# federicobetti99/Conjugate-Gradient

Measured on AMD Instinct MI355X. Metric: cg_iterations_per_sec, higher is better.
Workload: dtype f64

## Files before the change

conjugate-gradient_amd/cgx.py:

```python
import ctypes as C
import os
import subprocess
import sys

import numpy as np

_PKG = os.path.dirname(os.path.abspath(__file__))
LIB_PATH = os.path.join(_PKG, "libcgx.so")
UNIQUE_ID_BYTES = 128

IPC_HANDLE_BYTES = 64
COMM_SELF, COMM_LOOPBACK, COMM_RCCL, COMM_P2P = 0, 1, 2, 3
MATRIX_DENSE, MATRIX_BANDED = 0, 1
MATRIX_CSR = 2
MAX_DIAGONALS = 64

EXPORTS = [
    "cgx_config_init", "cgx_comm_unique_id", "cgx_create", "cgx_destroy", "cgx_last_error", "cgx_status_string",
    "cgx_get_comm_info", "cgx_get_gemv_plan", "cgx_get_resident_record", "cgx_p2p_export", "cgx_p2p_import", "cgx_p2p_selftest",
    "cgx_partition", "cgx_generate_lap2d_matrix", "cgx_set_matrix_dense", "cgx_read_matrix",
    "cgx_init_source_term", "cgx_set_source_term", "cgx_set_max_iter", "cgx_set_tolerance", "cgx_get_size",
    "cgx_get_matrix_format",
    "cgx_solve", "cgx_solve_begin", "cgx_solve_steps", "cgx_solve_end", "cgx_get_gemv_samples",
    "cgx_get_update_samples",
    "cgx_probe_gemv", "cgx_probe_time_gemv", "cgx_probe_vector_ops", "cgx_probe_get_matrix_rows",
    "cgx_probe_get_source_term", "cgx_probe_set_fault_after", "cgx_probe_set_resident_limit", "cgx_probe_persistent_plan",
    "cgx_probe_parse_matrix_market", "cgx_probe_p2p_mailbox_to_host", "cgx_probe_fill_matrix_hash",
    "cgx_probe_set_p2p_epoch", "cgx_probe_get_p2p_epoch", "cgx_probe_p2p_host_mailboxes", "cgx_probe_resident_test",
    "cgx_solve_multi", "cgx_probe_gemv_multi",
    "cgx_set_preconditioner", "cgx_get_preconditioner",
    "cgx_set_preconditioner_block", "cgx_get_preconditioner_block", "cgx_probe_get_precond_blocks",
    "cgx_set_matrix_csr", "cgx_get_matrix_nnz",
]
MAX_RHS = 16
PRECOND_NONE, PRECOND_JACOBI = 0, 1
_PRECOND_NAMES = {None: PRECOND_NONE, "jacobi": PRECOND_JACOBI}
PRECOND_BLOCKS = (1, 2, 4, 8, 16, 32, 64, 128, 256)


class Config(C.Structure):
    _fields_ = [
        ("struct_version", C.c_int), ("comm_mode", C.c_int), ("device", C.c_int), ("rank", C.c_int),
        ("nranks", C.c_int), ("unique_id", C.c_ubyte * UNIQUE_ID_BYTES), ("gemv_variant", C.c_int),
        ("lda_pad", C.c_int), ("check_every", C.c_int), ("profile_gemv", C.c_int), ("profile_update", C.c_int),
        ("p2p_mailbox_kib", C.c_int), ("p2p_timeout_ms", C.c_int), ("p2p_separate_exchange", C.c_int),
        ("matrix_format", C.c_int), ("profile_first", C.c_int), ("profile_markers", C.c_int),
        ("p2p_no_acquire_fence", C.c_int), ("p2p_tagged", C.c_int),
    ]


class Result(C.Structure):
    _fields_ = [
# ... 20 lines not shown
    subprocess.check_call(args)
    return LIB_PATH


_lib = None


def lib():
    global _lib
    if _lib is None:
        if not os.path.exists(LIB_PATH):
            raise OSError("libcgx.so not built (run `make -C conjugate-gradient_amd` or __graft_entry__.build()); "
                          "the product path has no CPU fallback")
        if "torch" not in sys.modules and os.environ.get("CGX_NO_TORCH") != "1":
            try:
                import torch
            except Exception:
                pass
        L = C.CDLL(LIB_PATH)
        dp = C.POINTER(C.c_double)
        ip = C.POINTER(C.c_int)
        vp = C.c_void_p
        L.cgx_config_init.argtypes = [C.POINTER(Config)]
        L.cgx_config_init.restype = None
        L.cgx_comm_unique_id.argtypes = [C.POINTER(C.c_ubyte)]
        L.cgx_create.argtypes = [C.POINTER(vp), C.POINTER(Config)]
        L.cgx_destroy.argtypes = [vp]
        L.cgx_last_error.argtypes = [vp]
        L.cgx_last_error.restype = C.c_char_p
        L.cgx_status_string.argtypes = [C.c_int]
        L.cgx_status_string.restype = C.c_char_p
        L.cgx_get_comm_info.argtypes = [vp, ip, ip, ip, C.c_char_p]
        L.cgx_get_gemv_plan.argtypes = [vp, C.c_int, ip]
        L.cgx_get_resident_record.argtypes = [vp, C.POINTER(C.c_longlong)]
        L.cgx_p2p_export.argtypes = [vp, C.POINTER(C.c_ubyte)]
        L.cgx_p2p_import.argtypes = [vp, C.POINTER(C.c_ubyte)]
        L.cgx_p2p_selftest.argtypes = [vp, C.c_int, ip]
        L.cgx_partition.argtypes = [C.c_int, C.c_int, ip, ip]
        L.cgx_generate_lap2d_matrix.argtypes = [vp, C.c_int]
        L.cgx_set_matrix_dense.argtypes = [vp, dp, C.c_long, C.c_int]
        L.cgx_read_matrix.argtypes = [vp, C.c_char_p]
        L.cgx_init_source_term.argtypes = [vp, C.c_double]
        L.cgx_set_source_term.argtypes = [vp, dp]
        L.cgx_set_max_iter.argtypes = [vp, C.c_int]
        L.cgx_set_tolerance.argtypes = [vp, C.c_double]
        L.cgx_get_size.argtypes = [vp, ip, ip]
        L.cgx_get_matrix_format.argtypes = [vp, C.c_int, ip, ip, ip, dp]
        L.cgx_set_matrix_csr.argtypes = [vp, C.c_int, C.POINTER(C.c_longlong), ip, dp]
        L.cgx_get_matrix_nnz.argtypes = [vp, C.c_int, C.POINTER(C.c_longlong)]
        L.cgx_solve.argtypes = [vp, dp, C.POINTER(Result)]
        L.cgx_solve_begin.argtypes = [vp, dp]
        L.cgx_solve_steps.argtypes = [vp, C.c_int, ip]
        L.cgx_solve_end.argtypes = [vp, dp, C.POINTER(Result)]
        L.cgx_get_gemv_samples.argtypes = [vp, dp, C.c_int, ip]
        L.cgx_get_update_samples.argtypes = [vp, dp, C.c_int, ip]
        L.cgx_probe_gemv.argtypes = [vp, dp, dp, dp]
        L.cgx_probe_time_gemv.argtypes = [vp, C.c_int, dp]
        L.cgx_probe_vector_ops.argtypes = [vp, C.c_int, C.c_double, C.c_double, dp, dp, dp, dp, dp]
        L.cgx_probe_get_matrix_rows.argtypes = [vp, C.c_int, dp, ip, ip]
        L.cgx_probe_get_source_term.argtypes = [vp, C.c_int, dp]
        L.cgx_probe_set_fault_after.argtypes = [vp, C.c_int]
        L.cgx_probe_set_resident_limit.argtypes = [vp, C.c_int]
        L.cgx_probe_persistent_plan.argtypes = [C.c_int, C.c_int, C.c_long, C.c_int, C.POINTER(C.c_long)]
        L.cgx_probe_p2p_mailbox_to_host.argtypes = [vp]
        L.cgx_probe_fill_matrix_hash.argtypes = [vp, C.c_ulonglong, C.c_int, C.c_double]
        L.cgx_probe_p2p_host_mailboxes.argtypes = [vp, C.c_char_p, C.c_int]
# ... 95 lines not shown
    def _check(self, st):
        if st:
            raise CgxError(st, lib().cgx_last_error(self._h).decode(errors="replace"))

    def close(self):
        if getattr(self, "_h", None) and self._h.value:
            lib().cgx_destroy(self._h)
            self._h = C.c_void_p()

    def __del__(self):
        try:
            self.close()
        except Exception:
            pass

    def __enter__(self):
        return self

    def __exit__(self, *exc):
        self.close()

    def comm_info(self):
        mode, wired, seen = C.c_int(), C.c_int(), C.c_int()
        dev = C.create_string_buffer(32)
        self._check(lib().cgx_get_comm_info(self._h, C.byref(mode), C.byref(wired), C.byref(seen), dev))
        return {"comm_mode": mode.value, "ranks_wired": wired.value, "rank_seen": seen.value,
                "device_id": dev.value.decode(errors="replace")}

    def gemv_plan(self, local_shard=0):
        v = (C.c_int * 8)()
        self._check(lib().cgx_get_gemv_plan(self._h, int(local_shard), v))
        return dict(zip(("variant", "R", "U", "waves", "light", "split", "grid", "ncols"), list(v)))

    def resident_record(self):
        v = (C.c_longlong * 10)()
        self._check(lib().cgx_get_resident_record(self._h, v))
        return dict(zip(("iterations", "watch_repeats", "gather_repeats", "launches", "wg0_first_wait_ticks", "wg0_longest_wait_ticks",
                         "max_first_wait_ticks", "max_longest_wait_ticks", "fallbacks", "persistent"), list(v)))

    def p2p_export(self):
        buf = (C.c_ubyte * IPC_HANDLE_BYTES)()
        self._check(lib().cgx_p2p_export(self._h, buf))
        return bytes(buf)

    def p2p_import(self, handles):
        assert len(handles) == self.nranks * IPC_HANDLE_BYTES
        buf = (C.c_ubyte * len(handles)).from_buffer_copy(handles)
        self._check(lib().cgx_p2p_import(self._h, buf))

    def p2p_selftest(self, rounds=32):
        ok = C.c_int()
        self._check(lib().cgx_p2p_selftest(self._h, int(rounds), C.byref(ok)))
        return bool(ok.value)

    def matrix_format(self, local_shard=0):
        fmt, nd, nbytes = C.c_int(), C.c_int(), C.c_double()
        offs = (C.c_int * MAX_DIAGONALS)()
        self._check(lib().cgx_get_matrix_format(self._h, int(local_shard), C.byref(fmt), C.byref(nd), offs, C.byref(nbytes)))
        return fmt.value, list(offs[:nd.value]), nbytes.value

    def matrix_nnz(self, local_shard=0):
        nnz = C.c_longlong()
        self._check(lib().cgx_get_matrix_nnz(self._h, int(local_shard), C.byref(nnz)))
        return nnz.value

    def set_matrix_csr(self, indptr, indices=None, data=None, n=None):
# ... 189 lines not shown
```

conjugate-gradient_amd/csrc/cgx_context.cpp:

```cpp
#include "cgx_internal.h"

#include <sys/mman.h>
#include <sys/stat.h>
#include <fcntl.h>
#include <unistd.h>

#include <algorithm>
#include <cctype>
#include <chrono>
#include <cmath>
#include <cstdio>
#include <cstdlib>
#include <cstring>
#include <string>
#include <vector>

using namespace cgxi;

namespace cgxi {

constexpr int kStreamDefaultMax = 10000;

thread_local std::string g_create_error;

// ... 25 lines not shown
void bind_state(Shard &s, long lda)
{
    double *b = s.state[s.cur];
    s.x = b;
    s.rbuf = b + cgx::state_off_r(lda);
    s.p[1] = b + cgx::state_off_p(lda);
    s.sc = reinterpret_cast<Scalars *>(b + cgx::state_off_sc(lda));
    s.rv.base = s.rbuf;
}

void free_shard(Shard &s)
{
    if (s.state[0]) {
        (void)hipFree(s.state[0]);
        (void)hipFree(s.state[1]);
        s.x = s.p[1] = s.rbuf = nullptr;
        s.sc = nullptr;
    }
    (void)hipFree(s.A);
    (void)hipFree(s.dia_vals);
    (void)hipFree(s.csr_rp);
    (void)hipFree(s.csr_col);
    (void)hipFree(s.csr_vals);
    (void)hipFree(s.b_full);
    (void)hipFree(s.x);
    (void)hipFree(s.p[0]);
    (void)hipFree(s.p[1]);
    (void)hipFree(s.apg);
    (void)hipFree(s.rbuf);
    (void)hipFree(s.partials);
    (void)hipFree(s.ap_parts);
    (void)hipFree(s.k1_scratch);
    (void)hipFree(s.sym_parts);
    (void)hipFree(s.dinv);
    (void)hipFree(s.W);
    (void)hipFree(s.zbuf);
    (void)hipFree(s.sc);
    (void)hipFree(s.gathered);
    s = Shard{};
}

void free_problem(cgx_ctx *ctx)
{
    for (auto &s : ctx->shards) free_shard(s);
    ctx->shards.clear();
    (void)hipFree(ctx->d_gathered_ptrs);
    (void)hipFree(ctx->d_scalar_ptrs);
    (void)hipFree(ctx->multi);
    ctx->multi = nullptr;
    ctx->multi_bytes = 0;
    if (ctx->h_stage) (void)hipHostFree(ctx->h_stage);
    ctx->h_stage = nullptr;
    ctx->d_gathered_ptrs = nullptr;
    ctx->d_scalar_ptrs = nullptr;
    ctx->have_matrix = ctx->have_b = false;
    ctx->in_solve = false;
    ctx->dinv_valid = false;
    (void)hipFree(ctx->d_jbad);
    ctx->d_jbad = nullptr;
}

static long p2p_flag_bytes() { return (long)cgx::kP2pChannels * cgx::kMaxRanks * cgx::kP2pFlagStride; }
static long p2p_data0_off() { return p2p_flag_bytes() + (long)cgx::kMaxChunkFlags * 8; }
long p2p_fixed_prefix(int nranks)
{
    return p2p_data0_off() + 2L * nranks * 16 + 2L * nranks * (long)cgx::kSlots * 8;
// ... 246 lines not shown
        }
        if (ctx->chunked) {
            HIP_TRY(ctx, hipMalloc(&s.k1_scratch, (size_t)(grid_max + 8) * sizeof(double)));
            HIP_TRY(ctx, hipMemsetAsync(s.k1_scratch, 0, (size_t)(grid_max + 8) * sizeof(double), ctx->stream));
        }
        if (!blocks) HIP_TRY(ctx, hipMalloc(&s.sc, sizeof(Scalars)));
        HIP_TRY(ctx, hipMalloc(&s.gathered, (size_t)cgx::kMaxRanks * cgx::kSlots * sizeof(double)));
        HIP_TRY(ctx, hipMemsetAsync(s.p[0], 0, (size_t)ctx->lda * sizeof(double), ctx->stream));
        HIP_TRY(ctx, hipMemsetAsync(s.p[1], 0, (size_t)ctx->lda * sizeof(double), ctx->stream));
        HIP_TRY(ctx, hipMemsetAsync(s.apg, 0, apg_bytes, ctx->stream));
        HIP_TRY(ctx, hipMemsetAsync(s.rbuf, 0, rbuf_bytes, ctx->stream));
        if (s.rows <= 0 && s.A) HIP_TRY(ctx, hipMemsetAsync(s.A, 0, (size_t)ctx->lda * sizeof(double), ctx->stream));
        HIP_TRY(ctx, hipMemsetAsync(s.partials, 0, (size_t)s.npartials * sizeof(double), ctx->stream));
        HIP_TRY(ctx, hipMemsetAsync(s.sc, 0, sizeof(Scalars), ctx->stream));
        HIP_TRY(ctx, hipMemsetAsync(s.gathered, 0, (size_t)cgx::kMaxRanks * cgx::kSlots * sizeof(double), ctx->stream));
    }
    CGX_TRY(setup_resident(ctx, variant));
    if (ctx->cfg.comm_mode == CGX_COMM_LOOPBACK) {
        std::vector<double *> gp(nlocal);
        std::vector<Scalars *> sp(nlocal);
        for (int i = 0; i < nlocal; ++i) {
            gp[i] = ctx->shards[i].gathered;
            sp[i] = ctx->shards[i].sc;
        }
        HIP_TRY(ctx, hipMalloc(&ctx->d_gathered_ptrs, nlocal * sizeof(double *)));
        HIP_TRY(ctx, hipMalloc(&ctx->d_scalar_ptrs, nlocal * sizeof(Scalars *)));
        HIP_TRY(ctx, hipMemcpy(ctx->d_gathered_ptrs, gp.data(), nlocal * sizeof(double *), hipMemcpyHostToDevice));
        HIP_TRY(ctx, hipMemcpy(ctx->d_scalar_ptrs, sp.data(), nlocal * sizeof(Scalars *), hipMemcpyHostToDevice));
    }
    HIP_TRY(ctx, hipStreamSynchronize(ctx->stream));
    return CGX_OK;
}

cgx_status plan_symmetric(cgx_ctx *ctx)
{
    ctx->dinv_valid = false;
    if (ctx->shards.size() != 1 || ctx->nranks != 1 || ctx->sparse() || ctx->chunked) return CGX_OK;
    Shard &s = ctx->shards[0];
    int variant = ctx->cfg.gemv_variant;
    if (variant <= 0) {
        const char *e = getenv("CGX_GEMV_VARIANT");
        if (e) variant = atoi(e);
    }
    const int k1_variant = (variant == 40000 || variant == 50000) ? 0 : variant;
    const cgx::GemvPlan general = cgx::plan_gemv(k1_variant, s.rows, ctx->n, ctx->lda, false);
    const cgx::GemvPlan sym = cgx::plan_symv(ctx->n, ctx->lda, ctx->cus);
    const bool eligible = variant <= 0 && ctx->n > cgx::kSymvMinN && s.rows == ctx->n && s.A && sym.light <= ctx->npart;
    if (!eligible) {
        s.plan = general;
        return CGX_OK;
    }
    DeviceScratch scratch;
    int *dflag = nullptr;
    HIP_TRY(ctx, scratch.alloc(&dflag, sizeof(int)));
    HIP_TRY(ctx, hipMemsetAsync(dflag, 0, sizeof(int), ctx->stream));
    HIP_TRY(ctx, cgx::launch_symmetric_check(s.A, ctx->lda, ctx->n, dflag, ctx->stream));
    int mismatch = 1;
    HIP_TRY(ctx, hipMemcpyAsync(&mismatch, dflag, sizeof(int), hipMemcpyDeviceToHost, ctx->stream));
    HIP_TRY(ctx, hipStreamSynchronize(ctx->stream));
    if (mismatch) {
        s.plan = general;
        return CGX_OK;
    }
    const size_t bytes = (size_t)sym.split * (size_t)ctx->lda * sizeof(double);
    if (s.sym_parts && s.sym_parts_bytes != bytes) {
        (void)hipFree(s.sym_parts);
        s.sym_parts = nullptr;
        s.sym_parts_bytes = 0;
    }
    if (!s.sym_parts) {
        HIP_TRY(ctx, hipMalloc(&s.sym_parts, bytes));
        s.sym_parts_bytes = bytes;
        HIP_TRY(ctx, hipMemsetAsync(s.sym_parts, 0, bytes, ctx->stream));
        HIP_TRY(ctx, hipStreamSynchronize(ctx->stream));
    }
    s.plan = sym;
    return CGX_OK;
}

}

extern "C" {

void cgx_config_init(cgx_config *cfg)
{
    if (!cfg) return;
    memset(cfg, 0, sizeof *cfg);
    cfg->struct_version = CGX_VERSION;
    cfg->comm_mode = CGX_COMM_SELF;
    cfg->device = 0;
    cfg->rank = 0;
    cfg->nranks = 1;
    cfg->lda_pad = -1;
}

const char *cgx_status_string(cgx_status s)
{
    switch (s) {
    case CGX_OK: return "ok";
    case CGX_ERR_BAD_ARG: return "bad argument";
    case CGX_ERR_IO: return "i/o error";
    case CGX_ERR_HIP: return "HIP error";
    case CGX_ERR_RCCL: return "RCCL error";
    case CGX_ERR_OOM: return "out of memory";
    case CGX_ERR_NO_DEVICE: return "no usable GPU (libcgx has no CPU fallback)";
    case CGX_ERR_UNSUPPORTED: return "unsupported input";
    case CGX_ERR_P2P: return "direct peer exchange failed";
    }
    return "unknown";
}
// ... 149 lines not shown
        break;
    case CGX_COMM_LOOPBACK:
        wired = ctx->nranks;
        break;
    default:
        break;
    }
    if (comm_mode) *comm_mode = ctx->cfg.comm_mode;
    if (ranks_wired) *ranks_wired = wired;
    if (rank_seen) *rank_seen = seen;
    if (device_id) {
        device_id[0] = 0;
        HIP_TRY(ctx, hipDeviceGetPCIBusId(device_id, 32, ctx->device));
    }
    return CGX_OK;
}

cgx_status cgx_get_gemv_plan(const cgx_ctx *ctx, int local_shard, int out[CGX_GEMV_PLAN_INTS])
{
    if (!ctx || !out || local_shard < 0 || local_shard >= (int)ctx->shards.size()) return CGX_ERR_BAD_ARG;
    const cgx::GemvPlan &pl = ctx->shards[(size_t)local_shard].plan;
    if (ctx->resident && ctx->rplan.stream) {
        const int r[CGX_GEMV_PLAN_INTS] = {5, ctx->rplan.R, ctx->rplan.S, 8, ctx->rplan.RB, ctx->rplan.RL + ctx->rplan.RG, ctx->rplan.grid, pl.ncols};
        memcpy(out, r, sizeof r);
        return CGX_OK;
    }
    if (ctx->resident) {
        const int r[CGX_GEMV_PLAN_INTS] = {4, ctx->rplan.R, ctx->rplan.S, 4, ctx->rplan.RG, 1, ctx->rplan.grid, pl.ncols};
        memcpy(out, r, sizeof r);
        return CGX_OK;
    }
    const int v[CGX_GEMV_PLAN_INTS] = {pl.variant, pl.R, pl.U, pl.waves, pl.light, pl.split, pl.grid, pl.ncols};
    memcpy(out, v, sizeof v);
    return CGX_OK;
}

cgx_status cgx_get_resident_record(const cgx_ctx *ctx, long long out[CGX_RESIDENT_RECORD_INTS])
{
    if (!ctx || !out) return CGX_ERR_BAD_ARG;
    for (int i = 0; i < 8; ++i) out[i] = ctx->res_rec[i];
    out[8] = ctx->res_fallbacks;
    out[9] = ctx->resident ? 1 : 0;
    return CGX_OK;
}

cgx_status cgx_p2p_export(cgx_ctx *ctx, unsigned char out[CGX_IPC_HANDLE_BYTES])
{
    static_assert(sizeof(hipIpcMemHandle_t) == CGX_IPC_HANDLE_BYTES, "hipIpcMemHandle_t size");
    if (!ctx || !out || ctx->cfg.comm_mode != CGX_COMM_P2P) return fail(ctx, CGX_ERR_BAD_ARG, "cgx_p2p_export: not a P2P context");
    HIP_TRY(ctx, hipSetDevice(ctx->device));
    hipIpcMemHandle_t h;
    HIP_TRY(ctx, hipIpcGetMemHandle(&h, ctx->mailbox));
    memcpy(out, &h, CGX_IPC_HANDLE_BYTES);
    return CGX_OK;
}

cgx_status cgx_p2p_import(cgx_ctx *ctx, const unsigned char *handles)
{
    if (!ctx || !handles || ctx->cfg.comm_mode != CGX_COMM_P2P) return fail(ctx, CGX_ERR_BAD_ARG, "cgx_p2p_import: not a P2P context");
    HIP_TRY(ctx, hipSetDevice(ctx->device));
    for (int q = 0; q < ctx->nranks; ++q) {
        if (q == ctx->cfg.rank) continue;
        hipIpcMemHandle_t h;
        memcpy(&h, handles + (size_t)q * CGX_IPC_HANDLE_BYTES, CGX_IPC_HANDLE_BYTES);
        void *ptr = nullptr;
        hipError_t e = hipIpcOpenMemHandle(&ptr, h, hipIpcMemLazyEnablePeerAccess);
// ... 216 lines not shown
```

conjugate-gradient_amd/csrc/cgx_internal.h:

```cpp
#pragma once

#include "../../include/cgx.h"

#include <hip/hip_runtime.h>

#include <string>
#include <vector>

#include "cgx_kernels.h"
#include "cgx_rccl.h"

namespace cgxi {

using cgx::Scalars;

struct Shard {
    int rank = 0;
    int row0 = 0;
    int rows = 0;
    double *A = nullptr;
    double *dia_vals = nullptr;
    cgx::DiaView dia{};
    long long *csr_rp = nullptr;
    int *csr_col = nullptr;
    double *csr_vals = nullptr;
    cgx::CsrView csr{};
    double *b_full = nullptr;
    double *state[2] = {nullptr, nullptr};
    int cur = 0;
    double *x = nullptr;
    double *p[2] = {nullptr, nullptr};
    double *apg = nullptr;
    double *rbuf = nullptr;
    double *ap_parts = nullptr;
    double *k1_scratch = nullptr;
    double *partials = nullptr;
    double *sym_parts = nullptr;
    size_t sym_parts_bytes = 0;
    Scalars *sc = nullptr;
    double *gathered = nullptr;
    cgx::GemvPlan plan{};
    cgx::SegView apv{}, rv{};
    double *dinv = nullptr;
    double *zbuf = nullptr;
    double *W = nullptr;
    int w_block = 0;
    cgx::SegView zv{};
    int npartials = 0;
    double *Ap() const { return apg + (size_t)rank * apv.S; }
    double *tail() const { return Ap() + apv.Sr; }
    double *k1_part() const { return k1_scratch ? k1_scratch : tail(); }
};


}

struct cgx_ctx {
    cgx_config cfg{};
    int device = 0;
    hipStream_t stream = nullptr;
    int nranks = 1;
    int m = 0, n = 0;
    long lda = 0;
    int max_iter = 0;
    double tol = 1e-10;
    std::vector<int> start_rows, num_rows;
    std::vector<cgxi::Shard> shards;
    std::vector<double> b_host;
    bool have_matrix = false, have_b = false;
    bool banded = false;
    bool csr = false;
// ... 192 lines not shown
```

conjugate-gradient_amd/csrc/cgx_kernels.h:

```cpp
#pragma once

#include <hip/hip_runtime.h>

namespace cgx {

constexpr int kSlots = 4;
constexpr int kSlotConj = 0;
constexpr int kSlotRr = 1;
constexpr int kSlotX = 2;
constexpr int kMaxRanks = 64;

struct Scalars {
    double rs[2];
    double rr[2];
    double local[kSlots];
    double dbg[4];
    int    done;
    int    k_final;
    unsigned pad[2];
};

struct SegView {
    double *base;
    int S, Sr;
// ... 8 lines not shown
void seg_finalize(SegView *sv);

struct GemvPlan {
    int variant;
    int R;
    int U;
    int waves;
    int nt;
    int grid;
    int rows_per_wg;
    int ncols;
    int split;
    int light;
};

GemvPlan plan_gemv(int variant, int rows, int n, long lda, bool allow_split = false);

hipError_t launch_gemv_plain(const GemvPlan &plan, const double *A, long lda, int rows, const double *v_full,
                             const double *v_local, double *Ap, double *partials, Scalars *sc, hipStream_t s);

hipError_t launch_gemv_fused(const GemvPlan &plan, const double *A, long lda, int rows, int row0,
                             const double *p_old, double *p_new, SegView seg, double *Ap, double *partials,
                             Scalars *sc, int k, double tol, hipStream_t s, hipEvent_t e_start = nullptr,
                             hipEvent_t e_stop = nullptr, long ap_stride = 0, bool jacobi = false);
constexpr int kSymvTile = 256;
constexpr int kSymvMinN = 16384;
GemvPlan plan_symv(int n, long lda, int cus);
inline int plan_partials(const GemvPlan &pl) { return pl.variant == 6 ? pl.light : pl.grid / (pl.split > 1 ? pl.split : 1); }
hipError_t launch_symv_plain(const GemvPlan &pl, const double *A, long lda, int n, const double *v, double *parts, double *Ap,
                             double *partials, hipStream_t s);
hipError_t launch_symv_fused(const GemvPlan &pl, const double *A, long lda, int n, const double *p_old, double *p_new, SegView seg,
                             double *parts, double *Ap, double *partials, Scalars *sc, int k, double tol, hipStream_t s,
                             hipEvent_t e_start = nullptr, hipEvent_t e_stop = nullptr, bool jacobi = false);
hipError_t launch_symmetric_check(const double *A, long lda, int n, int *mismatch, hipStream_t s);

constexpr int kChunkRows = 512;
inline int chunks_per_rank(int Sr) { return (Sr + kChunkRows - 1) / kChunkRows; }
hipError_t launch_prefold_ap(const double *parts, int split, long stride, int rows, int Sr, const double *p_loc, double *dst,
                             double *tail, const Scalars *sc, hipStream_t s);

hipError_t launch_update_xr(int n, int rows, int row0, const double *p_new, SegView apv, int tail_off, int tail_count,
                            double *x, SegView rv, Scalars *sc, int parity, double *partials, hipStream_t s,
                            hipEvent_t e_start = nullptr, hipEvent_t e_stop = nullptr,
                            const double *dinv = nullptr, SegView zv = SegView{},
                            const double *W = nullptr, int block = 1, long lda = 0);
int update_xr_grid(int count);
constexpr int kMaxVectorGrid = 1024;

hipError_t launch_close_iteration(Scalars *sc, SegView seg, int k, double tol, hipStream_t s, bool jacobi = false);

hipError_t launch_reduce_partials(const double *partials, int n, double *out, hipStream_t s);
hipError_t launch_reduce_partials3(const double *partials, int n, double *out3, hipStream_t s);

hipError_t launch_init_residual(int n, const double *b_full, SegView apv, SegView rv, double *partials, hipStream_t s,
                                const double *dinv = nullptr, SegView zv = SegView{}, const double *W = nullptr, int block = 1,
                                long lda = 0);

hipError_t launch_diag_slice(const double *A, long lda, int rows, int row0, double *dst, hipStream_t s);
hipError_t launch_jacobi_dinv(SegView apv, int n, long lda, double *dinv, int *bad, hipStream_t s);

constexpr int kBjMaxBlock = 256;
constexpr int kBjLdsBlock = 128;
bool bj_block_ok(int block);
hipError_t launch_bj_col_slice(const double *A, long lda, int n, int rows, int row0, int block, int t0, int nt, double *dst,
                               long dst_stride, hipStream_t s);
hipError_t launch_bj_invert(double *W, long lda, int n, int block, int *bad, hipStream_t s);
// ... 196 lines not shown
```

conjugate-gradient_amd/csrc/cgx_solve.cpp:

```cpp
#include "cgx_internal.h"

#include <sys/file.h>

#include <cerrno>
#include <climits>
#include <thread>

#include <algorithm>
#include <cctype>
#include <chrono>
#include <cmath>
#include <cstdio>
#include <cstdlib>
#include <cstring>
#include <string>
#include <vector>

using namespace cgxi;

namespace cgxi {


cgx_status p2p_allgather(cgx_ctx *ctx, int chan, const double *src, int count, double *dst, long dst_stride,
                         int copy_self, int tail_off, int tail_n, int sum_off)
// ... 175 lines not shown
    *out = ctx->ev_pool[ctx->ev_used++];
    return CGX_OK;
}

}

namespace {

cgx_status take_update_events(cgx_ctx *ctx, hipEvent_t *e0, hipEvent_t *e1)
{
    *e0 = *e1 = nullptr;
    if (!ctx->cfg.profile_update || !ctx->gemv_timed_last || ctx->cfg.profile_markers) return CGX_OK;
    while (ctx->upd_used + 2 > ctx->upd_pool.size()) {
        hipEvent_t e;
        HIP_TRY(ctx, hipEventCreate(&e));
        ctx->upd_pool.push_back(e);
    }
    *e0 = ctx->upd_pool[ctx->upd_used++];
    *e1 = ctx->upd_pool[ctx->upd_used++];
    return CGX_OK;
}

}

namespace cgxi {

cgx_status run_gemv_plain(cgx_ctx *ctx, Shard &s, const double *v_full)
{
    if (ctx->csr)
        HIP_TRY(ctx, cgx::launch_spmv_csr_plain(s.plan, s.csr, s.rows, s.row0, ctx->lda, v_full, s.Ap(), s.k1_part(), ctx->stream));
    else if (ctx->banded)
        HIP_TRY(ctx, cgx::launch_spmv_dia_plain(s.plan, s.dia, s.rows, s.row0, ctx->n, ctx->lda, v_full, s.Ap(), s.k1_part(), s.sc,
                                                ctx->stream));
    else if (s.plan.variant == 6)
        HIP_TRY(ctx, cgx::launch_symv_plain(s.plan, s.A, ctx->lda, ctx->n, v_full, s.sym_parts, s.Ap(), s.k1_part(), ctx->stream));
    else
        HIP_TRY(ctx, cgx::launch_gemv_plain(s.plan, s.A, ctx->lda, s.rows, v_full, v_full + s.row0, s.Ap(), s.k1_part(),
                                            s.sc, ctx->stream));
    return CGX_OK;
}

cgx_status run_gemv_fused(cgx_ctx *ctx, Shard &s, int k)
{
    const int every = ctx->cfg.profile_gemv;
    const long long seq = ctx->gemv_seq++;
    bool timed = false;
    if (every > 0 && ctx->ev_used + 2 <= 4096) {
        if (seq == 0) {
            timed = ctx->cfg.profile_first != 0;
            if (!timed) ctx->gemv_discarded++;
        } else {
            timed = ((seq - 1) % every) == 0;
        }
    }
    ctx->gemv_timed_last = timed;
    hipEvent_t e0 = nullptr, e1 = nullptr;
    if (timed) {
        CGX_TRY(take_event(ctx, &e0));
        CGX_TRY(take_event(ctx, &e1));
        if (ctx->cfg.profile_markers) {
            HIP_TRY(ctx, hipEventRecord(e0, ctx->stream));
            e0 = e1 = nullptr;
        }
    }
    hipEvent_t m1 = (timed && ctx->cfg.profile_markers) ? ctx->ev_pool[ctx->ev_used - 1] : nullptr;
    const bool pc = ctx->precond == CGX_PRECOND_JACOBI;
    if (ctx->csr)
        HIP_TRY(ctx, cgx::launch_spmv_csr_fused(s.plan, s.csr, s.rows, s.row0, ctx->lda, s.p[k & 1], s.p[(k + 1) & 1], pc ? s.zv : s.rv,
                                                s.Ap(), s.k1_part(), s.sc, k, ctx->tol, ctx->stream, e0, e1, pc));
    else if (ctx->banded)
        HIP_TRY(ctx, cgx::launch_spmv_dia_fused(s.plan, s.dia, s.rows, s.row0, ctx->n, ctx->lda, s.p[k & 1], s.p[(k + 1) & 1],
                                                s.rv, s.Ap(), s.k1_part(), s.sc, k, ctx->tol, ctx->stream, e0, e1));
    else if (s.plan.variant == 6)
        HIP_TRY(ctx, cgx::launch_symv_fused(s.plan, s.A, ctx->lda, ctx->n, s.p[k & 1], s.p[(k + 1) & 1], pc ? s.zv : s.rv, s.sym_parts,
                                            s.Ap(), s.k1_part(), s.sc, k, ctx->tol, ctx->stream, e0, e1, pc));
    else
        HIP_TRY(ctx, cgx::launch_gemv_fused(s.plan, s.A, ctx->lda, s.rows, s.row0, s.p[k & 1], s.p[(k + 1) & 1], pc ? s.zv : s.rv,
                                            s.plan.split > 1 ? s.ap_parts : s.Ap(),
                                            (ctx->chunked && s.plan.light) ? nullptr : s.k1_part(),
                                            s.sc, k, ctx->tol, ctx->stream, e0, e1, ctx->seg_Sr, pc));
    if (m1) HIP_TRY(ctx, hipEventRecord(m1, ctx->stream));
    return CGX_OK;
}

void reset_gemv_stats(cgx_ctx *ctx)
{
    ctx->ev_used = 0;
    ctx->gemv_ms_sum = ctx->gemv_ms_min = ctx->gemv_ms_max = 0;
    ctx->gemv_launches = ctx->gemv_discarded = 0;
    ctx->gemv_seq = 0;
    ctx->gemv_samples.clear();
    ctx->gemv_timed_last = false;
    ctx->upd_used = 0;
    ctx->upd_samples.clear();
    ctx->steps_ev_pending = false;
    ctx->steps_device_ms = 0;
}

cgx_status harvest_gemv_events(cgx_ctx *ctx)
{
    for (size_t i = 0; i + 1 < ctx->ev_used; i += 2) {
        float ms = 0.f;
        HIP_TRY(ctx, hipEventElapsedTime(&ms, ctx->ev_pool[i], ctx->ev_pool[i + 1]));
        ctx->gemv_ms_sum += ms;
        if (ctx->gemv_launches == 0 || ms < ctx->gemv_ms_min) ctx->gemv_ms_min = ms;
// ... 506 lines not shown
```

conjugate-gradient_amd/csrc/cgx_symv.hip:

```cpp
#include "cgx_kernels.h"
#include "cgx_device.h"

#include <hip/hip_ext.h>

namespace cgx {

__device__ __forceinline__ long strip_start(long I, long nb) { return I * nb - I * (I - 1) / 2; }
__device__ __forceinline__ void tri_tile(long t, long nb, long *I, long *J)
{
    const double b = 2.0 * (double)nb + 1.0;
    long i = (long)((b - sqrt(b * b - 8.0 * (double)t)) * 0.5);
    i = i < 0 ? 0 : (i > nb - 1 ? nb - 1 : i);
    while (i + 1 < nb && strip_start(i + 1, nb) <= t) ++i;
    while (i > 0 && strip_start(i, nb) > t) --i;
    *I = i;
    *J = i + (t - strip_start(i, nb));
}

template <int B, bool FUSED>
__global__ __launch_bounds__(256, 4) void k_symv_tiles(const double *__restrict__ A, long lda, int n, int ncols, int nb, long tiles,
                                                       const double *__restrict__ v, double *__restrict__ p_new, SegView sv,
                                                       double *__restrict__ parts, Scalars *sc, int k, double tol)
{
    constexpr bool PRE = false;
// ... 68 lines not shown
        }
        __syncthreads();
        bool bad = false;
#pragma unroll
        for (int y = y0; y < 32; y += 8) {
            const long r = I * 32 + y, c = J * 32 + x;
            if (r < n && c < n) bad |= Ab[r * lda + c] != tt[y][x];
        }
        if (bad) atomicOr(mismatch, 1);
        __syncthreads();
    }
}

GemvPlan plan_symv(int n, long lda, int cus)
{
    GemvPlan pl{};
    pl.variant = 6;
    pl.R = kSymvTile;
    pl.waves = 4;
    pl.nt = 1;
    pl.split = (n + kSymvTile - 1) / kSymvTile;
    const long tiles = (long)pl.split * (pl.split + 1) / 2;
    const long slots = 4L * (cus > 0 ? cus : 256);
    pl.grid = (int)(tiles < slots ? tiles : slots);
    pl.U = (int)((tiles + pl.grid - 1) / pl.grid);
    const int Sr = (n + 1) / 2 * 2;
    pl.light = (Sr + kFoldRows - 1) / kFoldRows;
    pl.ncols = (n + 1) & ~1;
    if (pl.ncols > (int)lda) pl.ncols = (int)lda;
    pl.rows_per_wg = kSymvTile;
    return pl;
}

namespace {

template <bool FUSED, bool PRE = false>
hipError_t launch_symv(const GemvPlan &pl, const double *A, long lda, int n, const double *v, double *p_new, SegView sv,
                       double *parts, double *Ap, double *tail, Scalars *sc, int k, double tol, hipStream_t s, hipEvent_t e0,
                       hipEvent_t e1)
{
    if (pl.variant != 6 || pl.R != kSymvTile || n < 2) return hipErrorInvalidValue;
    const long tiles = (long)pl.split * (pl.split + 1) / 2;
    if constexpr (PRE)
        hipExtLaunchKernelGGL((k_pcg_symv_tiles<kSymvTile>), dim3(pl.grid), dim3(256), 0, s, e0, nullptr, 0, A, lda, n, pl.ncols,
                              pl.split, tiles, v, p_new, sv, parts, sc, k, tol);
    else
        hipExtLaunchKernelGGL((k_symv_tiles<kSymvTile, FUSED>), dim3(pl.grid), dim3(256), 0, s, e0, nullptr, 0, A, lda, n, pl.ncols,
                              pl.split, tiles, v, p_new, sv, parts, sc, k, tol);
    hipError_t e = hipGetLastError();
    if (e != hipSuccess) return e;
    const int Sr = (n + 1) / 2 * 2;
    hipExtLaunchKernelGGL((k_symv_fold<FUSED>), dim3(pl.light), dim3(kFoldWaves * 64), 0, s, nullptr, e1, 0, parts, lda, pl.split, Sr,
                          FUSED ? p_new : v, Ap, tail, sc);
    return hipGetLastError();
}

}

hipError_t launch_symv_plain(const GemvPlan &pl, const double *A, long lda, int n, const double *v, double *parts, double *Ap,
                             double *partials, hipStream_t s)
{
    return launch_symv<false>(pl, A, lda, n, v, nullptr, SegView{}, parts, Ap, partials, nullptr, 0, 0.0, s, nullptr, nullptr);
}

hipError_t launch_symv_fused(const GemvPlan &pl, const double *A, long lda, int n, const double *p_old, double *p_new, SegView seg,
                             double *parts, double *Ap, double *partials, Scalars *sc, int k, double tol, hipStream_t s,
                             hipEvent_t e_start, hipEvent_t e_stop, bool jacobi)
{
    if (jacobi) return launch_symv<true, true>(pl, A, lda, n, p_old, p_new, seg, parts, Ap, partials, sc, k, tol, s, e_start, e_stop);
    return launch_symv<true>(pl, A, lda, n, p_old, p_new, seg, parts, Ap, partials, sc, k, tol, s, e_start, e_stop);
}

hipError_t launch_symmetric_check(const double *A, long lda, int n, int *mismatch, hipStream_t s)
{
    const long nt = ((long)n + 31) / 32, pairs = nt * (nt + 1) / 2;
    const long grid = pairs < 8192 ? pairs : 8192;
    hipLaunchKernelGGL(k_symmetric_check, dim3((unsigned)grid), dim3(256), 0, s, A, lda, n, nt, pairs, mismatch);
    return hipGetLastError();
}

}
```

include/cgx.h:

```cpp
#ifndef CGX_H
#define CGX_H

#ifdef __cplusplus
extern "C" {
#endif

#define CGX_VERSION 1
#define CGX_UNIQUE_ID_BYTES 128
#define CGX_IPC_HANDLE_BYTES 64

typedef enum cgx_status {
    CGX_OK = 0,
    CGX_ERR_BAD_ARG = 1,
    CGX_ERR_IO = 2,
    CGX_ERR_HIP = 3,
    CGX_ERR_RCCL = 4,
    CGX_ERR_OOM = 5,
    CGX_ERR_NO_DEVICE = 6,
    CGX_ERR_UNSUPPORTED = 7,
    CGX_ERR_P2P = 8
} cgx_status;

typedef enum cgx_comm_mode {
    CGX_COMM_SELF = 0,
// ... 34 lines not shown
typedef struct cgx_result {
    int    iterations;
    int    converged;
    double residual_prev;
    double residual_last;
    double x_norm;
    double rel_residual;
    double seconds_solve;
    double seconds_loop;
    double gemv_ms_avg;
    double gemv_ms_min;
    long long gemv_launches;
    double gemv_bytes;
    double gemv_ms_median;
    double gemv_ms_max;
    long long gemv_discarded;
    double steps_device_ms;
} cgx_result;

typedef struct cgx_ctx cgx_ctx;

void        cgx_config_init(cgx_config *cfg);
cgx_status  cgx_comm_unique_id(unsigned char out[CGX_UNIQUE_ID_BYTES]);
cgx_status  cgx_create(cgx_ctx **out, const cgx_config *cfg);
cgx_status  cgx_destroy(cgx_ctx *ctx);
const char *cgx_last_error(const cgx_ctx *ctx);
const char *cgx_status_string(cgx_status s);

cgx_status  cgx_get_comm_info(cgx_ctx *ctx, int *comm_mode, int *ranks_wired, int *rank_seen, char *device_id);

#define CGX_GEMV_PLAN_INTS 8
cgx_status  cgx_get_gemv_plan(const cgx_ctx *ctx, int local_shard, int out[CGX_GEMV_PLAN_INTS]);

#define CGX_RESIDENT_RECORD_INTS 10
cgx_status  cgx_get_resident_record(const cgx_ctx *ctx, long long out[CGX_RESIDENT_RECORD_INTS]);

cgx_status  cgx_p2p_export(cgx_ctx *ctx, unsigned char out[CGX_IPC_HANDLE_BYTES]);
cgx_status  cgx_p2p_import(cgx_ctx *ctx, const unsigned char *handles);
cgx_status  cgx_p2p_selftest(cgx_ctx *ctx, int rounds, int *ok);

cgx_status  cgx_partition(int n, int psize, int *start_rows, int *num_rows);

cgx_status  cgx_generate_lap2d_matrix(cgx_ctx *ctx, int size);
cgx_status  cgx_set_matrix_dense(cgx_ctx *ctx, const double *A, long lda, int n);
cgx_status  cgx_read_matrix(cgx_ctx *ctx, const char *mtx_path);
cgx_status  cgx_set_matrix_csr(cgx_ctx *ctx, int n, const long long *row_ptr, const int *col_idx, const double *vals);
cgx_status  cgx_init_source_term(cgx_ctx *ctx, double h);
cgx_status  cgx_set_source_term(cgx_ctx *ctx, const double *b );
cgx_status  cgx_set_max_iter(cgx_ctx *ctx, int max_iter);
cgx_status  cgx_set_tolerance(cgx_ctx *ctx, double tol);
cgx_status  cgx_get_size(const cgx_ctx *ctx, int *m, int *n);
#define CGX_PRECOND_NONE 0
#define CGX_PRECOND_JACOBI 1
cgx_status  cgx_set_preconditioner(cgx_ctx *ctx, int kind);
cgx_status  cgx_get_preconditioner(const cgx_ctx *ctx, int *kind);
cgx_status  cgx_set_preconditioner_block(cgx_ctx *ctx, int block);
cgx_status  cgx_get_preconditioner_block(const cgx_ctx *ctx, int *block);
cgx_status  cgx_get_matrix_format(const cgx_ctx *ctx, int local_shard, int *format, int *ndiag, int *offsets,
                                  double *matrix_bytes);
cgx_status  cgx_get_matrix_nnz(const cgx_ctx *ctx, int local_shard, long long *nnz);

cgx_status  cgx_solve(cgx_ctx *ctx, double *x, cgx_result *res);

cgx_status  cgx_solve_begin(cgx_ctx *ctx, const double *x0);
cgx_status  cgx_solve_steps(cgx_ctx *ctx, int nsteps, int *done_out);
cgx_status  cgx_solve_end(cgx_ctx *ctx, double *x, cgx_result *res);
// ... 33 lines not shown
```

Baseline: 1491.

## Pack upper-triangular symmetric tiles contiguously for the symv path

Adds a one-time packing kernel that copies the upper-triangular B×B tiles of the dense symmetric matrix into a contiguous tile-major buffer. New tri-tile kernels (plain and fused CG variants) stream these packed tiles linearly, so each workgroup reads sequential memory instead of strided rows of the full matrix, then reuse the existing fold kernel. The intent is better DRAM streaming efficiency for the bandwidth-bound symmetric matvec. The cost is an extra matrix-sized allocation of roughly half the dense matrix, held alongside it, plus a pack step during planning. It is on by default and can be disabled with an environment variable.

```diff
diff --git a/conjugate-gradient_amd/cgx.py b/conjugate-gradient_amd/cgx.py
--- a/conjugate-gradient_amd/cgx.py
+++ b/conjugate-gradient_amd/cgx.py
@@ -17,7 +17,7 @@
 
 EXPORTS = [
     "cgx_config_init", "cgx_comm_unique_id", "cgx_create", "cgx_destroy", "cgx_last_error", "cgx_status_string",
-    "cgx_get_comm_info", "cgx_get_gemv_plan", "cgx_get_resident_record", "cgx_p2p_export", "cgx_p2p_import", "cgx_p2p_selftest",
+    "cgx_get_comm_info", "cgx_get_gemv_plan", "cgx_get_symv_storage", "cgx_get_resident_record", "cgx_p2p_export", "cgx_p2p_import", "cgx_p2p_selftest",
     "cgx_partition", "cgx_generate_lap2d_matrix", "cgx_set_matrix_dense", "cgx_read_matrix",
     "cgx_init_source_term", "cgx_set_source_term", "cgx_set_max_iter", "cgx_set_tolerance", "cgx_get_size",
     "cgx_get_matrix_format",
@@ -104,6 +104,7 @@
         L.cgx_status_string.restype = C.c_char_p
         L.cgx_get_comm_info.argtypes = [vp, ip, ip, ip, C.c_char_p]
         L.cgx_get_gemv_plan.argtypes = [vp, C.c_int, ip]
+        L.cgx_get_symv_storage.argtypes = [vp, ip, C.POINTER(C.c_ulonglong)]
         L.cgx_get_resident_record.argtypes = [vp, C.POINTER(C.c_longlong)]
         L.cgx_p2p_export.argtypes = [vp, C.POINTER(C.c_ubyte)]
         L.cgx_p2p_import.argtypes = [vp, C.POINTER(C.c_ubyte)]
@@ -265,6 +266,11 @@
         self._check(lib().cgx_get_gemv_plan(self._h, int(local_shard), v))
         return dict(zip(("variant", "R", "U", "waves", "light", "split", "grid", "ncols"), list(v)))
 
+    def symv_storage(self):
+        packed, nbytes = C.c_int(0), C.c_ulonglong(0)
+        self._check(lib().cgx_get_symv_storage(self._h, C.byref(packed), C.byref(nbytes)))
+        return packed.value, nbytes.value
+
     def resident_record(self):
         v = (C.c_longlong * 10)()
         self._check(lib().cgx_get_resident_record(self._h, v))
diff --git a/conjugate-gradient_amd/csrc/cgx_context.cpp b/conjugate-gradient_amd/csrc/cgx_context.cpp
--- a/conjugate-gradient_amd/csrc/cgx_context.cpp
+++ b/conjugate-gradient_amd/csrc/cgx_context.cpp
@@ -81,6 +81,7 @@
     (void)hipFree(s.ap_parts);
     (void)hipFree(s.k1_scratch);
     (void)hipFree(s.sym_parts);
+    (void)hipFree(s.sym_packed);
     (void)hipFree(s.dinv);
     (void)hipFree(s.W);
     (void)hipFree(s.zbuf);
@@ -393,6 +394,20 @@
     return CGX_OK;
 }
 
+static void drop_packed(Shard &s)
+{
+    (void)hipFree(s.sym_packed);
+    s.sym_packed = nullptr;
+    s.sym_packed_bytes = 0;
+}
+
+static cgx_status pack_tiles(cgx_ctx *ctx, Shard &s)
+{
+    HIP_TRY(ctx, cgx::launch_tri_pack(s.A, ctx->lda, ctx->n, s.sym_packed, ctx->stream));
+    HIP_TRY(ctx, hipStreamSynchronize(ctx->stream));
+    return CGX_OK;
+}
+
 cgx_status plan_symmetric(cgx_ctx *ctx)
 {
     ctx->dinv_valid = false;
@@ -409,6 +424,7 @@
     const bool eligible = variant <= 0 && ctx->n > cgx::kSymvMinN && s.rows == ctx->n && s.A && sym.light <= ctx->npart;
     if (!eligible) {
         s.plan = general;
+        if (s.sym_packed) drop_packed(s);
         return CGX_OK;
     }
     DeviceScratch scratch;
@@ -421,11 +437,13 @@
     HIP_TRY(ctx, hipStreamSynchronize(ctx->stream));
     if (mismatch) {
         s.plan = general;
+        if (s.sym_packed) drop_packed(s);
         return CGX_OK;
     }
     const size_t bytes = (size_t)sym.split * (size_t)ctx->lda * sizeof(double);
     if (s.sym_parts && s.sym_parts_bytes != bytes) {
         (void)hipFree(s.sym_parts);
+    (void)hipFree(s.sym_packed);
         s.sym_parts = nullptr;
         s.sym_parts_bytes = 0;
     }
@@ -436,7 +454,27 @@
         HIP_TRY(ctx, hipStreamSynchronize(ctx->stream));
     }
     s.plan = sym;
-    return CGX_OK;
+    const char *pk = getenv("CGX_SYMV_PACKED");
+    const size_t pbytes = (pk && atoi(pk) == 0) ? 0 : cgx::tri_packed_bytes(ctx->n);
+    if (s.sym_packed && s.sym_packed_bytes != pbytes) drop_packed(s);
+    if (!pbytes) return CGX_OK;
+    if (!s.sym_packed) {
+        const hipError_t me = fault_due(ctx) ? hipErrorUnknown : hipMalloc(&s.sym_packed, pbytes);
+        if (me == hipErrorOutOfMemory) {
+            (void)hipGetLastError();
+            s.sym_packed = nullptr;
+            return CGX_OK;
+        }
+        if (me != hipSuccess) {
+            s.sym_packed = nullptr;
+            quiesce(ctx);
+            return fail(ctx, CGX_ERR_HIP, std::string("hipMalloc(sym_packed): ") + hipGetErrorString(me));
+        }
+        s.sym_packed_bytes = pbytes;
+    }
+    const cgx_status st = pack_tiles(ctx, s);
+    if (st != CGX_OK) drop_packed(s);
+    return st;
 }
 
 }
@@ -652,6 +690,15 @@
     }
     const int v[CGX_GEMV_PLAN_INTS] = {pl.variant, pl.R, pl.U, pl.waves, pl.light, pl.split, pl.grid, pl.ncols};
     memcpy(out, v, sizeof v);
+    return CGX_OK;
+}
+
+cgx_status cgx_get_symv_storage(const cgx_ctx *ctx, int *packed, unsigned long long *bytes)
+{
+    if (!ctx || !packed || !bytes) return CGX_ERR_BAD_ARG;
+    const bool on = ctx->shards.size() == 1 && ctx->shards[0].plan.variant == 6 && ctx->shards[0].sym_packed;
+    *packed = on ? 1 : 0;
+    *bytes = on ? (unsigned long long)ctx->shards[0].sym_packed_bytes : 0ull;
     return CGX_OK;
 }
 
diff --git a/conjugate-gradient_amd/csrc/cgx_internal.h b/conjugate-gradient_amd/csrc/cgx_internal.h
--- a/conjugate-gradient_amd/csrc/cgx_internal.h
+++ b/conjugate-gradient_amd/csrc/cgx_internal.h
@@ -37,6 +37,8 @@
     double *partials = nullptr;
     double *sym_parts = nullptr;
     size_t sym_parts_bytes = 0;
+    double *sym_packed = nullptr;
+    size_t sym_packed_bytes = 0;
     Scalars *sc = nullptr;
     double *gathered = nullptr;
     cgx::GemvPlan plan{};
diff --git a/conjugate-gradient_amd/csrc/cgx_kernels.h b/conjugate-gradient_amd/csrc/cgx_kernels.h
--- a/conjugate-gradient_amd/csrc/cgx_kernels.h
+++ b/conjugate-gradient_amd/csrc/cgx_kernels.h
@@ -64,6 +64,15 @@
 hipError_t launch_symv_fused(const GemvPlan &pl, const double *A, long lda, int n, const double *p_old, double *p_new, SegView seg,
                              double *parts, double *Ap, double *partials, Scalars *sc, int k, double tol, hipStream_t s,
                              hipEvent_t e_start = nullptr, hipEvent_t e_stop = nullptr, bool jacobi = false);
+hipError_t launch_symv_fold(const GemvPlan &pl, long lda, int n, const double *parts, const double *p, double *Ap, double *tail,
+                            const Scalars *sc, hipStream_t s, hipEvent_t e_stop = nullptr);
+size_t tri_packed_bytes(int n);
+hipError_t launch_tri_pack(const double *A, long lda, int n, double *At, hipStream_t s);
+hipError_t launch_tri_plain(const GemvPlan &pl, const double *At, long lda, int n, const double *v, double *parts, double *Ap,
+                            double *partials, hipStream_t s);
+hipError_t launch_tri_fused(const GemvPlan &pl, const double *At, long lda, int n, const double *p_old, double *p_new, SegView seg,
+                            double *parts, double *Ap, double *partials, Scalars *sc, int k, double tol, hipStream_t s,
+                            hipEvent_t e_start = nullptr, hipEvent_t e_stop = nullptr, bool jacobi = false);
 hipError_t launch_symmetric_check(const double *A, long lda, int n, int *mismatch, hipStream_t s);
 
 constexpr int kChunkRows = 512;
diff --git a/conjugate-gradient_amd/csrc/cgx_solve.cpp b/conjugate-gradient_amd/csrc/cgx_solve.cpp
--- a/conjugate-gradient_amd/csrc/cgx_solve.cpp
+++ b/conjugate-gradient_amd/csrc/cgx_solve.cpp
@@ -231,6 +231,8 @@
     else if (ctx->banded)
         HIP_TRY(ctx, cgx::launch_spmv_dia_plain(s.plan, s.dia, s.rows, s.row0, ctx->n, ctx->lda, v_full, s.Ap(), s.k1_part(), s.sc,
                                                 ctx->stream));
+    else if (s.plan.variant == 6 && s.sym_packed)
+        HIP_TRY(ctx, cgx::launch_tri_plain(s.plan, s.sym_packed, ctx->lda, ctx->n, v_full, s.sym_parts, s.Ap(), s.k1_part(), ctx->stream));
     else if (s.plan.variant == 6)
         HIP_TRY(ctx, cgx::launch_symv_plain(s.plan, s.A, ctx->lda, ctx->n, v_full, s.sym_parts, s.Ap(), s.k1_part(), ctx->stream));
     else
@@ -270,6 +272,9 @@
     else if (ctx->banded)
         HIP_TRY(ctx, cgx::launch_spmv_dia_fused(s.plan, s.dia, s.rows, s.row0, ctx->n, ctx->lda, s.p[k & 1], s.p[(k + 1) & 1],
                                                 s.rv, s.Ap(), s.k1_part(), s.sc, k, ctx->tol, ctx->stream, e0, e1));
+    else if (s.plan.variant == 6 && s.sym_packed)
+        HIP_TRY(ctx, cgx::launch_tri_fused(s.plan, s.sym_packed, ctx->lda, ctx->n, s.p[k & 1], s.p[(k + 1) & 1], pc ? s.zv : s.rv, s.sym_parts,
+                                           s.Ap(), s.k1_part(), s.sc, k, ctx->tol, ctx->stream, e0, e1, pc));
     else if (s.plan.variant == 6)
         HIP_TRY(ctx, cgx::launch_symv_fused(s.plan, s.A, ctx->lda, ctx->n, s.p[k & 1], s.p[(k + 1) & 1], pc ? s.zv : s.rv, s.sym_parts,
                                             s.Ap(), s.k1_part(), s.sc, k, ctx->tol, ctx->stream, e0, e1, pc));
diff --git a/conjugate-gradient_amd/csrc/cgx_symv.hip b/conjugate-gradient_amd/csrc/cgx_symv.hip
--- a/conjugate-gradient_amd/csrc/cgx_symv.hip
+++ b/conjugate-gradient_amd/csrc/cgx_symv.hip
@@ -124,6 +124,19 @@
     return pl;
 }
 
+hipError_t launch_symv_fold(const GemvPlan &pl, long lda, int n, const double *parts, const double *p, double *Ap, double *tail,
+                            const Scalars *sc, hipStream_t s, hipEvent_t e1)
+{
+    const int Sr = (n + 1) / 2 * 2;
+    if (sc)
+        hipExtLaunchKernelGGL((k_symv_fold<true>), dim3(pl.light), dim3(kFoldWaves * 64), 0, s, nullptr, e1, 0, parts, lda, pl.split, Sr,
+                              p, Ap, tail, sc);
+    else
+        hipExtLaunchKernelGGL((k_symv_fold<false>), dim3(pl.light), dim3(kFoldWaves * 64), 0, s, nullptr, e1, 0, parts, lda, pl.split, Sr,
+                              p, Ap, tail, sc);
+    return hipGetLastError();
+}
+
 namespace {
 
 template <bool FUSED, bool PRE = false>
@@ -141,10 +154,7 @@
                               pl.split, tiles, v, p_new, sv, parts, sc, k, tol);
     hipError_t e = hipGetLastError();
     if (e != hipSuccess) return e;
-    const int Sr = (n + 1) / 2 * 2;
-    hipExtLaunchKernelGGL((k_symv_fold<FUSED>), dim3(pl.light), dim3(kFoldWaves * 64), 0, s, nullptr, e1, 0, parts, lda, pl.split, Sr,
-                          FUSED ? p_new : v, Ap, tail, sc);
-    return hipGetLastError();
+    return launch_symv_fold(pl, lda, n, parts, FUSED ? p_new : v, Ap, tail, FUSED ? sc : nullptr, s, e1);
 }
 
 }
diff --git a/conjugate-gradient_amd/csrc/cgx_tri.hip b/conjugate-gradient_amd/csrc/cgx_tri.hip
--- /dev/null
+++ b/conjugate-gradient_amd/csrc/cgx_tri.hip
@@ -0,0 +1,111 @@
+#include "cgx_kernels.h"
+#include "cgx_device.h"
+
+#include <hip/hip_ext.h>
+
+namespace cgx {
+
+namespace {
+
+__device__ __forceinline__ long tri_strip_start(long I, long nb) { return I * nb - I * (I - 1) / 2; }
+__device__ __forceinline__ void tri_tile_of(long t, long nb, long *I, long *J)
+{
+    const double b = 2.0 * (double)nb + 1.0;
+    long i = (long)((b - sqrt(b * b - 8.0 * (double)t)) * 0.5);
+    i = i < 0 ? 0 : (i > nb - 1 ? nb - 1 : i);
+    while (i + 1 < nb && tri_strip_start(i + 1, nb) <= t) ++i;
+    while (i > 0 && tri_strip_start(i, nb) > t) --i;
+    *I = i;
+    *J = i + (t - tri_strip_start(i, nb));
+}
+
+__device__ __forceinline__ void tri_slot_store(double *dst, double v)
+{
+#if defined(CGX_TRI_SLOT_NT) && CGX_TRI_SLOT_NT
+    __builtin_nontemporal_store(v, dst);
+#else
+    *dst = v;
+#endif
+}
+
+}
+
+template <int B>
+__global__ __launch_bounds__(256) void k_tri_pack(const double *__restrict__ A, long lda, int n, int nb, long tiles,
+                                                  double *__restrict__ At)
+{
+    constexpr int PER = B / 2;
+    constexpr int ROWS = 256 / PER;
+    static_assert(256 % PER == 0 && B % ROWS == 0, "tile shape");
+    const int piece = threadIdx.x % PER, rs = threadIdx.x / PER;
+    for (long t = blockIdx.x; t < tiles; t += gridDim.x) {
+        long I, J;
+        tri_tile_of(t, nb, &I, &J);
+        const long col = J * B + 2 * piece;
+        d2 *dst = reinterpret_cast<d2 *>(At + t * (long)(B * B)) + piece;
+#pragma unroll 8
+        for (int r = rs; r < B; r += ROWS) {
+            const long row = I * B + r;
+            d2 x{0.0, 0.0};
+            if (row < n && col < n) x = *reinterpret_cast<const d2 *>(A + row * lda + col);
+            __builtin_nontemporal_store(x, dst + (long)r * PER);
+        }
+    }
+}
+
+template <int B, bool FUSED, bool PRE>
+__global__ __launch_bounds__(256, 4) void k_tri_tiles(const double *__restrict__ At, long lda, int n, int ncols, int nb, long tiles,
+                                                      const double *__restrict__ v, double *__restrict__ p_new, SegView sv,
+                                                      double *__restrict__ parts, Scalars *sc, int k, double tol)
+{
+    static_assert(FUSED || !PRE, "the Jacobi form is fused only");
+#include "cgx_tri_tiles.inc"
+}
+
+size_t tri_packed_bytes(int n)
+{
+    const size_t nb = ((size_t)n + kSymvTile - 1) / kSymvTile;
+    return nb * (nb + 1) / 2 * (size_t)kSymvTile * kSymvTile * sizeof(double);
+}
+
+hipError_t launch_tri_pack(const double *A, long lda, int n, double *At, hipStream_t s)
+{
+    if (n < 2 || !A || !At) return hipErrorInvalidValue;
+    const long nb = ((long)n + kSymvTile - 1) / kSymvTile, tiles = nb * (nb + 1) / 2;
+    hipLaunchKernelGGL((k_tri_pack<kSymvTile>), dim3((unsigned)tiles), dim3(256), 0, s, A, lda, n, (int)nb, tiles, At);
+    return hipGetLastError();
+}
+
+namespace {
+
+template <bool FUSED, bool PRE = false>
+hipError_t launch_tri(const GemvPlan &pl, const double *At, long lda, int n, const double *v, double *p_new, SegView sv,
+                      double *parts, double *Ap, double *tail, Scalars *sc, int k, double tol, hipStream_t s, hipEvent_t e0,
+                      hipEvent_t e1)
+{
+    if (pl.variant != 6 || pl.R != kSymvTile || n < 2 || !At) return hipErrorInvalidValue;
+    const long tiles = (long)pl.split * (pl.split + 1) / 2;
+    hipExtLaunchKernelGGL((k_tri_tiles<kSymvTile, FUSED, PRE>), dim3(pl.grid), dim3(256), 0, s, e0, nullptr, 0, At, lda, n, pl.ncols,
+                          pl.split, tiles, v, p_new, sv, parts, sc, k, tol);
+    const hipError_t e = hipGetLastError();
+    if (e != hipSuccess) return e;
+    return launch_symv_fold(pl, lda, n, parts, FUSED ? p_new : v, Ap, tail, FUSED ? sc : nullptr, s, e1);
+}
+
+}
+
+hipError_t launch_tri_plain(const GemvPlan &pl, const double *At, long lda, int n, const double *v, double *parts, double *Ap,
+                            double *partials, hipStream_t s)
+{
+    return launch_tri<false>(pl, At, lda, n, v, nullptr, SegView{}, parts, Ap, partials, nullptr, 0, 0.0, s, nullptr, nullptr);
+}
+
+hipError_t launch_tri_fused(const GemvPlan &pl, const double *At, long lda, int n, const double *p_old, double *p_new, SegView seg,
+                            double *parts, double *Ap, double *partials, Scalars *sc, int k, double tol, hipStream_t s,
+                            hipEvent_t e_start, hipEvent_t e_stop, bool jacobi)
+{
+    if (jacobi) return launch_tri<true, true>(pl, At, lda, n, p_old, p_new, seg, parts, Ap, partials, sc, k, tol, s, e_start, e_stop);
+    return launch_tri<true>(pl, At, lda, n, p_old, p_new, seg, parts, Ap, partials, sc, k, tol, s, e_start, e_stop);
+}
+
+}
diff --git a/conjugate-gradient_amd/csrc/cgx_tri_tiles.inc b/conjugate-gradient_amd/csrc/cgx_tri_tiles.inc
--- /dev/null
+++ b/conjugate-gradient_amd/csrc/cgx_tri_tiles.inc
@@ -0,0 +1,101 @@
+    constexpr int H = B / 128;
+    constexpr int R = 16 / H;
+    constexpr int RW = B / 4;
+    static_assert(H >= 1 && RW % R == 0 && RW <= 64, "tile shape");
+    __shared__ double rowbuf[2][B];
+    __shared__ double colbuf[2][4][B];
+
+    const int lane = threadIdx.x & 63, w = threadIdx.x >> 6;
+    const long G = gridDim.x, bid = blockIdx.x;
+    const long q = tiles / G, rem = tiles - q * G;
+    const long t0 = bid * q + (bid < rem ? bid : rem), t1 = t0 + q + (bid < rem ? 1 : 0);
+    double beta = 0.0;
+    if constexpr (FUSED) {
+        const HeadLoadsOf<PRE> hl = head_issue_t<PRE>(sc, sv, k);
+        const IterHead h = head_finish_t<PRE>(hl, sc, sv, k, tol);
+        if (hl.done || h.stop) return;
+        beta = h.beta;
+    }
+    if (t0 >= t1) return;
+    long I, J;
+    tri_tile_of(t0, nb, &I, &J);
+    const double *rfull = sv.base;
+
+    auto vec2 = [&](int c) {
+        const bool ok = c < ncols;
+        const int cc = ok ? c : 0;
+        d2 p = *reinterpret_cast<const d2 *>(v + cc);
+        if constexpr (FUSED) {
+            const d2 r = *reinterpret_cast<const d2 *>(rfull + cc);
+            p.x = fma(beta, p.x, r.x);
+            p.y = fma(beta, p.y, r.y);
+        }
+        p.x = ok ? p.x : 0.0;
+        p.y = ok ? p.y : 0.0;
+        return p;
+    };
+    auto vec1 = [&](int i) {
+        const bool ok = i < n;
+        const int ii = ok ? i : 0;
+        double p = v[ii];
+        if constexpr (FUSED) p = fma(beta, p, rfull[ii]);
+        return ok ? p : 0.0;
+    };
+
+    const double *tp = At + t0 * (long)(B * B) + (long)(w * RW) * B + 2 * lane;
+    int buf = 0;
+    for (long t = t0; t < t1; ++t, tp += B * B) {
+        const int r0 = (int)(I * B), c0 = (int)(J * B);
+        const bool diag = I == J;
+        d2 pj[H];
+#pragma unroll
+        for (int h = 0; h < H; ++h) {
+            const int col = c0 + h * 128 + 2 * lane;
+            pj[h] = vec2(col);
+            if constexpr (FUSED)
+                if (diag && w == 0 && col < ncols) *reinterpret_cast<d2 *>(p_new + col) = pj[h];
+        }
+        const double pi_l = vec1(r0 + w * RW + (lane & (RW - 1)));
+        d2 cacc[H];
+#pragma unroll
+        for (int h = 0; h < H; ++h) cacc[h] = d2{0.0, 0.0};
+
+        for (int b = 0; b < RW / R; ++b) {
+            const double *bp = tp + (long)(b * R) * B;
+            d2 a[R][H];
+#pragma unroll
+            for (int q2 = 0; q2 < R; ++q2)
+#pragma unroll
+                for (int h = 0; h < H; ++h) a[q2][h] = load_a<true>(bp + q2 * B + h * 128);
+            __builtin_amdgcn_sched_barrier(0);
+            double racc[R];
+#pragma unroll
+            for (int q2 = 0; q2 < R; ++q2) {
+                racc[q2] = fma(a[q2][0].y, pj[0].y, a[q2][0].x * pj[0].x);
+#pragma unroll
+                for (int h = 1; h < H; ++h) racc[q2] = fma(a[q2][h].y, pj[h].y, fma(a[q2][h].x, pj[h].x, racc[q2]));
+                const int src = b * R + q2;
+                const double pr = __hiloint2double(__builtin_amdgcn_readlane(__double2hiint(pi_l), src),
+                                                   __builtin_amdgcn_readlane(__double2loint(pi_l), src));
+#pragma unroll
+                for (int h = 0; h < H; ++h) {
+                    cacc[h].x = fma(a[q2][h].x, pr, cacc[h].x);
+                    cacc[h].y = fma(a[q2][h].y, pr, cacc[h].y);
+                }
+            }
+            const int myrow = wave_sum_rows<R>(racc, lane);
+            if ((lane & (64 / R - 1)) == 0) rowbuf[buf][w * RW + b * R + myrow] = racc[0];
+        }
+        if (!diag)
+#pragma unroll
+            for (int h = 0; h < H; ++h) *reinterpret_cast<d2 *>(&colbuf[buf][w][h * 128 + 2 * lane]) = cacc[h];
+        __syncthreads();
+        for (int e = threadIdx.x; e < B; e += 256) {
+            if (r0 + e < n) tri_slot_store(parts + J * lda + r0 + e, rowbuf[buf][e]);
+            if (!diag && c0 + e < n)
+                tri_slot_store(parts + I * lda + c0 + e,
+                               ((colbuf[buf][0][e] + colbuf[buf][1][e]) + colbuf[buf][2][e]) + colbuf[buf][3][e]);
+        }
+        buf ^= 1;
+        if (++J == nb) { ++I; J = I; }
+    }
diff --git a/include/cgx.h b/include/cgx.h
--- a/include/cgx.h
+++ b/include/cgx.h
@@ -90,6 +90,8 @@
 #define CGX_GEMV_PLAN_INTS 8
 cgx_status  cgx_get_gemv_plan(const cgx_ctx *ctx, int local_shard, int out[CGX_GEMV_PLAN_INTS]);
 
+cgx_status  cgx_get_symv_storage(const cgx_ctx *ctx, int *packed, unsigned long long *bytes);
+
 #define CGX_RESIDENT_RECORD_INTS 10
 cgx_status  cgx_get_resident_record(const cgx_ctx *ctx, long long out[CGX_RESIDENT_RECORD_INTS]);
 
```

Result: slower. 1347 (-9.6%).
